# SaumikDana/Bayesian-Markov-chain-Monte-Carlo

Hardware: AMD Instinct MI355X
Metric: ode_steps_x_chains_per_sec (higher is better)
Workload: dtype f64

## Files before the change

### bayesian-markov-chain-monte-carlo_amd/csrc/rsf_device.h

```cpp
#pragma once
#include <hip/hip_runtime.h>
#include <stdint.h>

#include <type_traits>

#include "rsf_math.h"

namespace rsf {

struct Consts {
  double mu_ref, V_ref, k1, mu0;
  double a_def, b_def;
  double h, hh, h6;
  double inv_dt;
  double t0, dt;
  double inv_vref;
  double cacc;
  const double *vl;
  const double *data;
  int64_t group_chains;
  int32_t nout;
  int32_t S;
  int32_t kc;
  int32_t nchunks;
};

__device__ __forceinline__ void select_group(Consts &K) {
  if (K.group_chains > 0) K.data += ((int64_t)blockIdx.x * blockDim.x / K.group_chains) * K.nout;
}

struct Lane {
  double inv_dc;
  double vdc;
  double kprime;
  double kia;
  double khh, kh, kh6;
  double vk;
  double beta;
  double kvk;
  double vrw;
  double hhdw, hdw;
  double cv;
  double h6v;
  double boa;
  double nhboa;
  double tc;
  double hhd, hd, h6d;
  double bh;
  double c_l1p, c_l1q;
  double c_em1;
};

template <int T>
__device__ __forceinline__ void set_tier(Lane &L);

template <bool DAMP>
__device__ __forceinline__ Lane make_lane(double dc, double a, double b, const Consts &K) {
  Lane L;
  const double inv_a = fm::rcp(a);
  L.inv_dc = fm::rcp(dc);
  L.kprime = (1e-2 * 10) * L.inv_dc;
  L.kia = L.kprime * inv_a;
  L.khh = L.kia * K.hh;
  L.kh = L.kia * K.h;
  L.kh6 = L.kia * K.h6;
  const double via = K.V_ref * inv_a;
  L.vdc = K.V_ref * L.inv_dc;
  L.vk = via * L.kprime;
  L.beta = (b * K.V_ref) * (1.0 / (1e-2 * 10));
  L.kvk = K.k1 * via;
  const double ikw = DAMP ? fm::rcp(L.kvk) : 1.0;
  const double vkw = DAMP ? L.vk * ikw : L.vk;
  L.cv = K.cacc * vkw;
  L.h6v = K.h6 * vkw;
  L.boa = b * inv_a;
  L.tc = -K.mu_ref * inv_a;
  L.hhd = K.hh * L.vdc;
  L.hd = K.h * L.vdc;
  L.h6d = K.h6 * L.vdc;
  L.vrw = DAMP ? K.V_ref * ikw : K.V_ref;
  L.hhdw = DAMP ? L.hhd * ikw : L.hhd;
  L.hdw = DAMP ? L.hd * ikw : L.hd;
  L.nhboa = -0.5 * L.boa;
  L.bh = L.beta * fm::rcp(L.hhd);
  set_tier<2>(L);
  return L;
}


struct State {
  double ms, x, V;
  double w, rx;
};

template <bool DAMP>
__device__ __forceinline__ void rhs_tail(double w, double rx, double x, double vl, const Lane &L,
                                         const Consts &K, double &d0, double &d1, double &d2) {
  d1 = __builtin_fma(-w, x, 1.0);
  d0 = __builtin_fma(-K.V_ref, w, vl);
  const double bt = (L.beta * d1) * rx;
  double g = d0 - bt;
  if (DAMP) {
    const double kw = L.kvk * w;
    d0 = __builtin_fma(-kw, g, d0);
    g = d0 - bt;
    d2 = kw * g;
  } else {
    d2 = w * g;
  }
}

__device__ __forceinline__ void eval_full(double ms, double x, const Lane &L, const Consts &K, double &w, double &rx) {
  w = fm::exp(__builtin_fma(-L.boa, fm::log(x), __builtin_fma(ms, L.kia, L.tc)));
  rx = fm::rcp(x);
}

enum Tier : int { TIGHT = 0, NARROW = 1, WIDE = 2, FULL = 3 };

__device__ __forceinline__ double local_value(double x) {
  asm volatile("" : "+v"(x));
  return x;
}

template <bool DAMP, int T>
__device__ __forceinline__ void tier_enter(State &s, const Lane &L) {
  s.rx *= L.hhd;
  if (DAMP) s.w *= L.kvk;
}
template <int T>
__device__ __forceinline__ void tier_x(State &s, const Lane &L) { s.x = L.hhd * fm::rcp(s.rx); }
template <bool DAMP, int T>
__device__ __forceinline__ void tier_leave(State &s, const Lane &L) {
  tier_x<T>(s, L);
  s.rx *= fm::rcp(local_value(L.hhd));
  if (DAMP) s.w *= fm::rcp(local_value(L.kvk));
}
template <bool DAMP, int T>
__device__ __forceinline__ void eval_full_t(State &s, const Lane &L, const Consts &K) {
  eval_full(s.ms, s.x, L, K, s.w, s.rx);
  tier_enter<DAMP, T>(s, L);
}
template <bool DAMP, int T>
__device__ __forceinline__ void resync_t(State &s, const Lane &L, const Consts &K) {
  tier_x<T>(s, L);
  eval_full_t<DAMP, T>(s, L, K);
}


struct Guard {
  float rho, dlt;
  float dlt_h;
};

__device__ __forceinline__ float hi_as_float(double x) { return __builtin_bit_cast(float, __double2hiint(x)); }
constexpr float hi_pow2(int e) { return __builtin_bit_cast(float, (1023 + e) << 20); }


template <int T>
__device__ __forceinline__ void set_tier(Lane &L) {
  L.c_l1p = L.boa * (1.0 / 3.0);
  L.c_l1q = L.boa * (-1.0 / 4.0);
  L.c_em1 = T == TIGHT ? 1.0 / 24.0 : (T == NARROW ? 1.0 / 720.0 : 1.0 / 40320.0);
  asm volatile("" : "+v"(L.c_l1p), "+v"(L.c_l1q), "+v"(L.c_em1));
}

template <int T>
__device__ __forceinline__ bool guard_ok(const Guard &g) {
  return (g.rho < (T == WIDE ? hi_pow2(-11) : (T == NARROW ? hi_pow2(-14) : hi_pow2(-20)))) &&
         (g.dlt < (T == TIGHT ? hi_pow2(-9) : (T == NARROW ? hi_pow2(-7) : hi_pow2(-5)))) && (T != TIGHT || g.dlt_h < hi_pow2(-10));
}

constexpr float hi_pow2_34(int e) { return __builtin_bit_cast(float, ((1023 + e - 1) << 20) | 0x80000); }
template <int T>
__device__ __forceinline__ bool calm_enough(const Guard &g) {
  static_assert(T == NARROW || T == WIDE, "TIGHT has no tighter tier");
  return T == WIDE ? (g.rho < hi_pow2_34(-14) && g.dlt < hi_pow2_34(-7))
                   : (g.rho < hi_pow2_34(-20) && g.dlt < hi_pow2_34(-10));
}

constexpr int kResync = 512;

template <bool DAMP>
__device__ __forceinline__ double rk4_cold(State &s, double vl0, double vlm, double vl1, const Lane &L,
                                           const Consts &K) {
  double k0 = 0.0, k1 = 0.0, s0 = 0.0, s1 = 0.0, s2 = 0.0;
#pragma nounroll
  for (int st = 0; st < 4; ++st) {
    const double c = st == 0 ? 0.0 : (st == 3 ? K.h : K.hh);
    const double wgt = (st == 0 || st == 3) ? 1.0 : 2.0;
    const double vl = st == 0 ? vl0 : (st == 3 ? vl1 : vlm);
    const double x1 = __builtin_fma(c * L.vdc, k1, s.x);
    double w, rx, d0, d1, d2;
    eval_full(__builtin_fma(c, k0, s.ms), x1, L, K, w, rx);
    rhs_tail<DAMP>(w, rx, x1, vl, L, K, d0, d1, d2);
    s0 = __builtin_fma(wgt, d0, s0);
    s1 = __builtin_fma(wgt, d1, s1);
    s2 = __builtin_fma(wgt, d2, s2);
    k0 = d0;
    k1 = d1;
  }
  s.ms = __builtin_fma(K.h6, s0, s.ms);
  s.x = __builtin_fma(L.h6d, s1, s.x);
  return s2;
}

template <int T, bool HALF>
__device__ __forceinline__ void tight_incr(double rho, double dk, const Lane &L, double w0, double &w, double &q, Guard &g) {
  g.rho = __builtin_fmaxf(g.rho, __builtin_fabsf(hi_as_float(rho)));
  double pb = L.nhboa;
  if (T == NARROW) pb = __builtin_fma(rho, L.c_l1p, pb);
  if (T == WIDE) pb = __builtin_fma(rho, __builtin_fma(rho, L.c_l1q, L.c_l1p), pb);
  const double dlt = __builtin_fma(-rho, __builtin_fma(rho, pb, L.boa), dk);
  if (T == TIGHT && HALF) g.dlt_h = __builtin_fmaxf(g.dlt_h, __builtin_fabsf(hi_as_float(dlt)));
  else g.dlt = __builtin_fmaxf(g.dlt, __builtin_fabsf(hi_as_float(dlt)));
  double e = L.c_em1;
  if (T == WIDE) {
    e = fm::hfma(e, dlt, 1.0 / 5040.0);
    e = fm::hfma(e, dlt, 1.0 / 720.0);
  }
  if (T != TIGHT) {
    e = fm::hfma(e, dlt, 1.0 / 120.0);
    e = fm::hfma(e, dlt, 1.0 / 24.0);
  }
  e = fm::hfma(e, dlt, 1.0 / 6.0);
  e = __builtin_fma(e, dlt, 0.5);
  e = __builtin_fma(e, dlt, 1.0);
  w = __builtin_fma(w0 * dlt, e, w0);
  const double r1 = __builtin_fma(rho, rho, -rho);
  q = r1;
  if (T != TIGHT) q = __builtin_fma(-rho, q, -rho);
  if (T == WIDE) q = __builtin_fma(-rho, q, -rho);
}

template <bool DAMP>
__device__ __forceinline__ void rhs_tight(double w, double xr, double Rh, double vl, double brx, double vr, double &d0, double &d1,
                                          double &g) {
  d1 = __builtin_fma(-w, xr, Rh);
  d0 = __builtin_fma(-vr, w, vl);
  g = __builtin_fma(-brx, d1, d0);
  if (DAMP) {
    d0 = __builtin_fma(-w, g, d0);
    g = __builtin_fma(-w, g, g);
  }
}

template <bool DAMP, int T>
__device__ __forceinline__ double rk4_tight(State &s, double vl0, double vlm, double vl1, const Lane &L, const Consts &K, Guard &g) {
  double a0, a1, a2, b0, b1, b2, c0, c1, c2, e0, e1, e2, w, q;
  const double Rh = s.rx;
  const double vr = L.vrw, xh = L.hhdw, xf = L.hdw;
  rhs_tight<DAMP>(s.w, xh, Rh, vl0, L.bh, vr, a0, a1, a2);
  double sv = s.w * a2;
  tight_incr<T, true>(a1, L.khh * a0, L, s.w, w, q, g);
  rhs_tight<DAMP>(w, __builtin_fma(xh, a1, xh), Rh, vlm, __builtin_fma(L.bh, q, L.bh), vr, b0, b1, b2);
  double sm = w * b2;
  tight_incr<T, true>(b1, L.khh * b0, L, s.w, w, q, g);
  rhs_tight<DAMP>(w, __builtin_fma(xh, b1, xh), Rh, vlm, __builtin_fma(L.bh, q, L.bh), vr, c0, c1, c2);
  sm = __builtin_fma(w, c2, sm);
  tight_incr<T, false>(c1 + c1, L.kh * c0, L, s.w, w, q, g);
  rhs_tight<DAMP>(w, __builtin_fma(xf, c1, xh), Rh, vl1, __builtin_fma(L.bh, q, L.bh), vr, e0, e1, e2);
  sv = __builtin_fma(w, e2, sv);
  const double t0 = a0 + 2.0 * b0 + 2.0 * c0 + e0;
  const double t1 = a1 + 2.0 * b1 + 2.0 * c1 + e1;
  const double rho = t1 * (1.0 / 3.0);
  tight_incr<T, false>(rho, L.kh6 * t0, L, s.w, w, q, g);
  s.ms = __builtin_fma(K.h6, t0, s.ms);
  s.w = w;
  s.rx = __builtin_fma(Rh, q, Rh);
  return __builtin_fma(2.0, sm, sv);
}

__device__ __forceinline__ State initial_state(double dc, const Lane &L, const Consts &K) {
  State s;
  s.ms = (K.mu0 * dc) * (1.0 / (1e-2 * 10));
  s.x = K.V_ref * ((dc * K.inv_vref) * L.inv_dc);
  s.V = K.V_ref;
  eval_full(s.ms, s.x, L, K, s.w, s.rx);
  return s;
}

constexpr int kLdsPad = 0;
__device__ __forceinline__ int lds_data_offset(const Consts &K) { return 2 * K.S * K.kc + 1 + kLdsPad; }
__device__ __forceinline__ int lds_d0_offset(const Consts &K) { return lds_data_offset(K) + K.kc; }

__device__ __forceinline__ void stage_chunk(double *lds, const Consts &K, int k0, int kn) {
  const int nv = 2 * K.S * kn + 1;
  const int base = 2 * K.S * (k0 - 1);
  __syncthreads();
  for (int i = threadIdx.x; i < nv; i += blockDim.x) lds[i] = K.vl[base + i];
  if (K.data) {
    double *ld = lds + lds_data_offset(K);
    for (int i = threadIdx.x; i < kn; i += blockDim.x) ld[i] = K.data[k0 + i];
    if (threadIdx.x == 0) lds[lds_d0_offset(K)] = K.data[0];
  }
  __syncthreads();
}

struct Emit {
  int ko;
  int phase;
  double vprev;
};

template <bool WANT_SSQ, bool WANT_ACC>
__device__ __forceinline__ void emit_at(double vnow, double vprev, int ko, double obs, const Consts &K, int k0,
                                        double &ssq, bool active, double *acc_out, int64_t stride) {
  const double ak = (vnow - vprev) * K.inv_dt;
  if (WANT_ACC && active) acc_out[(int64_t)(k0 + ko) * stride] = ak;
  if (WANT_SSQ) {
    const double r = ak - obs;
    ssq = __builtin_fma(r, r, ssq);
  }
}

template <bool WANT_SSQ, bool WANT_ACC>
__device__ __forceinline__ void emit_incr(double dvs, int ko, double obs, const Lane &L, int k0, double &ssq,
                                          bool active, double *acc_out, int64_t stride) {
  if (WANT_ACC && active) acc_out[(int64_t)(k0 + ko) * stride] = dvs * L.cv;
  if (WANT_SSQ) {
    const double r = __builtin_fma(dvs, L.cv, -obs);
    ssq = __builtin_fma(r, r, ssq);
  }
}

template <bool WANT_SSQ, bool WANT_ACC>
__device__ __forceinline__ void emit_sample(double vnow, Emit &em, double obs, const Consts &K, int k0, double &ssq,
                                            bool active, double *acc_out, int64_t stride) {
  emit_at<WANT_SSQ, WANT_ACC>(vnow, em.vprev, em.ko, obs, K, k0, ssq, active, acc_out, stride);
  em.vprev = vnow;
  ++em.ko;
}

template <bool DAMP, int T, int NU>
__device__ __forceinline__ bool trip_fast(const double *v, const Lane &L, const Consts &K, State &s, double (&dv)[NU], bool *calm = nullptr) {
  Guard g = {0, 0, 0};
#pragma unroll
  for (int j = 0; j < NU; ++j) dv[j] = rk4_tight<DAMP, T>(s, v[2 * j], v[2 * j + 1], v[2 * j + 2], L, K, g);
  if constexpr (T != TIGHT) {
    if (calm) *calm = calm_enough<T>(g);
  }
  return !guard_ok<T>(g);
}

template <bool DAMP, int T, int NU>
__device__ __forceinline__ void trip_cold(const double *v, const Lane &L, const Consts &K, State &s, double (&dv)[NU]) {
  tier_x<T>(s, L);
#pragma unroll 1
  for (int j = 0; j < NU; ++j) {
    const double r = rk4_cold<DAMP>(s, v[2 * j], v[2 * j + 1], v[2 * j + 2], L, K);
#pragma unroll
    for (int m = 0; m < NU; ++m) dv[m] = m == j ? r : dv[m];
  }
  eval_full_t<DAMP, T>(s, L, K);
}

template <bool DAMP, int NU>
__device__ __forceinline__ void trip_cold_plain(const double *v, const Lane &L, const Consts &K, State &s, double (&dv)[NU]) {
#pragma unroll 1
  for (int j = 0; j < NU; ++j) {
    const double r = rk4_cold<DAMP>(s, v[2 * j], v[2 * j + 1], v[2 * j + 2], L, K);
#pragma unroll
    for (int m = 0; m < NU; ++m) dv[m] = m == j ? r : dv[m];
  }
  eval_full(s.ms, s.x, L, K, s.w, s.rx);
}

constexpr int kFullRetry = 32;
constexpr int kCalmSteps = 16;
struct Wave {
  unsigned long long alive;
  unsigned long long need[3];
  unsigned long long stiff;
  int next_resync;
  int full_run;
  int calm;
  uint32_t steps[4], redone, lane_steps;
};

__device__ __forceinline__ unsigned long long ballot(bool p) { return __builtin_amdgcn_ballot_w64(p); }
__device__ __forceinline__ bool lane_in(unsigned long long mask) { return (mask >> (threadIdx.x & 63)) & 1; }
template <int CTRL>
__device__ __forceinline__ double dpp_move(double v) {
  const int lo = __builtin_amdgcn_update_dpp(0, __double2loint(v), CTRL, 0xF, 0xF, false);
  const int hi = __builtin_amdgcn_update_dpp(0, __double2hiint(v), CTRL, 0xF, 0xF, false);
  return __hiloint2double(hi, lo);
}

__device__ __forceinline__ void wave_begin(Wave &W, bool active, const Lane &L, const Consts &K) {
  const double dk = 1.2 * K.V_ref * K.h * L.kia;
  W.alive = ballot(active);
  W.need[0] = ballot(active && !(dk < 0x1.0p-9));
  W.need[1] = ballot(active && !(dk < 0x1.0p-7));
  W.need[2] = W.stiff = ballot(active && !(dk < 0x1.0p-3));
  W.next_resync = kResync;
  W.full_run = 0;
  W.calm = 0;
}

__device__ __forceinline__ int wave_tier(const Wave &W) {
  return (W.need[2] & W.alive) ? FULL : ((W.need[1] & W.alive) ? WIDE : ((W.need[0] & W.alive) ? NARROW : TIGHT));
}

template <bool WANT_SSQ, bool WANT_ACC, bool S1, int NU>
__device__ __forceinline__ void emit_trip(const double (&dv)[NU], const double (&obs)[NU], const double *ld, int r, State &s, Emit &em,
                                          const Lane &L, const Consts &K, int k0, double &ssq, bool active, double *acc_out, int64_t stride) {
  if (S1) {
#pragma unroll
    for (int j = 0; j < NU; ++j) emit_incr<WANT_SSQ, WANT_ACC>(dv[j], r + j, obs[j], L, k0, ssq, active, acc_out, stride);
  } else {
#pragma unroll
    for (int j = 0; j < NU; ++j) {
      s.V = __builtin_fma(L.h6v, dv[j], s.V);
      if (++em.phase == K.S) {
        em.phase = 0;
        const double o = WANT_SSQ ? ld[em.ko] : 0.0;
        emit_sample<WANT_SSQ, WANT_ACC>(s.V, em, o, K, k0, ssq, active, acc_out, stride);
      }
    }
  }
}

constexpr int kTightUnroll = 8;
constexpr int kNarrowUnroll = 8, kWiderUnroll = 4;
template <bool DAMP, bool WANT_SSQ, bool WANT_ACC, int T, bool S1, int NU>
__device__ __forceinline__ int integrate_multi(const double *lds, const double *ld, const Consts &K, Lane L, int k0, int kn, int r,
                                               int nsteps, State &s, Emit &em, double &ssq, double thr, bool active, double *acc_out,
                                               int64_t stride, Wave &W) {
  static_assert(NU >= 1 && (kResync % NU) == 0, "trip lengths divide the resync interval");
  set_tier<T>(L);
  for (; r + NU <= nsteps; r += NU) {
    const unsigned long long deadmask = WANT_SSQ ? ballot(ssq > thr) : 0ull;
    const double *v = lds + 2 * r;
    double obs[NU], dv[NU];
#pragma unroll
    for (int j = 0; j < NU; ++j) obs[j] = (WANT_SSQ && S1) ? ld[r + j] : 0.0;
    if (r >= W.next_resync) {
      resync_t<DAMP, T>(s, L, K);
      W.next_resync = (r & ~(kResync - 1)) + kResync;
    }
    const State save = s;
    bool calm = false;
    const bool bad = trip_fast<DAMP, T, NU>(v, L, K, s, dv, &calm);
    const unsigned long long badmask = ballot(bad) & W.alive;
    W.steps[T] += NU;
    W.lane_steps += NU * (uint32_t)__builtin_popcountll(W.alive);
    if constexpr (T != TIGHT) {
      W.calm = (ballot(!calm) & W.alive) == 0 ? W.calm + NU : 0;
    }
    if (__builtin_expect(badmask != 0, 0)) {
      if (lane_in(badmask)) {
        s = save;
        trip_cold<DAMP, T, NU>(v, L, K, s, dv);
      }
      W.need[T] |= badmask;
      W.redone += NU;
      W.full_run = 0;
      W.calm = 0;
    }
    emit_trip<WANT_SSQ, WANT_ACC, S1, NU>(dv, obs, ld, r, s, em, L, K, k0, ssq, active, acc_out, stride);
    W.alive &= ~deadmask;
    if constexpr (T != TIGHT) {
      if (W.calm >= kCalmSteps && badmask == 0) {
        W.need[T - 1] &= ~W.alive | W.stiff;
        W.calm = 0;
      }
    }
    if (badmask != 0 || W.alive == 0 || (T != TIGHT && (W.need[T - 1] & W.alive) == 0)) return r + NU;
  }
  return r;
}

template <bool DAMP, bool WANT_SSQ, bool WANT_ACC, bool S1>
__device__ __forceinline__ int integrate_full(const double *lds, const double *ld, const Consts &K, const Lane &L, int k0, int kn, int r,
                                              int nsteps, State &s, Emit &em, double &ssq, double thr, bool active, double *acc_out,
                                              int64_t stride, Wave &W) {
#pragma unroll 1
  for (; r < nsteps; ++r) {
    const unsigned long long deadmask = WANT_SSQ ? ballot(ssq > thr) : 0ull;
    const double *v = lds + 2 * r;
    const double obs[1] = {(WANT_SSQ && S1) ? ld[r] : 0.0};
    const double dv[1] = {rk4_cold<DAMP>(s, v[0], v[1], v[2], L, K)};
    W.steps[FULL] += 1;
    W.lane_steps += (uint32_t)__builtin_popcountll(W.alive);
    emit_trip<WANT_SSQ, WANT_ACC, S1, 1>(dv, obs, ld, r, s, em, L, K, k0, ssq, active, acc_out, stride);
    W.alive &= ~deadmask;
    if (++W.full_run >= kFullRetry) {
      W.need[2] &= W.stiff;
      W.full_run = 0;
    }
    if (W.alive == 0 || (W.need[2] & W.alive) == 0) return r + 1;
  }
  return r;
}

__device__ __forceinline__ int start_tier(const Lane &L, const Consts &K) {
  const double dk = 1.2 * K.V_ref * K.h * L.kia;
  return !__any(!(dk < 0x1.0p-9)) ? TIGHT : (!__any(!(dk < 0x1.0p-7)) ? NARROW : WIDE);
}

constexpr int kLockstepTrip = 8;
template <bool DAMP, typename OnSample, typename AfterTrip>
__device__ __forceinline__ void integrate_lockstep(double *lds, const Consts &K, const Lane &L, State &st, int kn, OnSample on_sample,
                                                   AfterTrip after_trip) {
  constexpr int NU = kLockstepTrip;
  static_assert(kResync % NU == 0, "the resync test looks at the first step of a trip");
  const int nsteps = K.S * kn;
  double dsum = 0.0;
  int phase = 0, ko = 0;
  int tier = start_tier(L, K);
  int r = 0;
  auto trip = [&](auto tier_tag, auto nu_tag) {
    constexpr int T = decltype(tier_tag)::value, NUT = decltype(nu_tag)::value;
    const double *v = lds + 2 * r;
    Lane Lt = L;
    set_tier<T>(Lt);
    const State save = st;
    double dv[NUT];
    tier_enter<DAMP, T>(st, Lt);
    const bool bad = trip_fast<DAMP, T, NUT>(v, Lt, K, st, dv);
    tier_leave<DAMP, T>(st, Lt);
    const bool any_bad = ballot(bad) != 0;
    if (__builtin_expect(any_bad, 0)) {
      if (bad) {
        st = save;
        trip_cold_plain<DAMP, NUT>(v, L, K, st, dv);
      }
    }
#pragma unroll
    for (int j = 0; j < NUT; ++j) {
      dsum += dv[j];
      if (++phase == K.S) {
        phase = 0;
        on_sample(dsum * L.cv, ko);
        dsum = 0.0;
        ++ko;
      }
    }
    return any_bad;
  };
  for (; r + NU <= nsteps; r += NU) {
    if ((r & (kResync - 1)) == 0) eval_full(st.ms, st.x, L, K, st.w, st.rx);
    bool any_bad;
    if (tier == TIGHT) any_bad = trip(std::integral_constant<int, TIGHT>{}, std::integral_constant<int, NU>{});
    else if (tier == NARROW) any_bad = trip(std::integral_constant<int, NARROW>{}, std::integral_constant<int, NU>{});
    else any_bad = trip(std::integral_constant<int, WIDE>{}, std::integral_constant<int, NU>{});
    if (any_bad && tier < WIDE) ++tier;
    after_trip();
  }
  for (; r < nsteps; ++r) {
    if ((r & (kResync - 1)) == 0) eval_full(st.ms, st.x, L, K, st.w, st.rx);
    trip(std::integral_constant<int, WIDE>{}, std::integral_constant<int, 1>{});
    after_trip();
  }
}

template <bool DAMP, bool WANT_SSQ, bool WANT_ACC, int T, bool S1, int NU>
__device__ __forceinline__ int integrate_tier(const double *lds, const double *ld, const Consts &K, const Lane &L, int k0, int kn, int r,
                                              int nsteps, State &s, Emit &em, double &ssq, double thr, bool active, double *acc_out,
                                              int64_t stride, Wave &W) {
  if (r + NU <= nsteps) return integrate_multi<DAMP, WANT_SSQ, WANT_ACC, T, S1, NU>(lds, ld, K, L, k0, kn, r, nsteps, s, em, ssq, thr, active, acc_out, stride, W);
  return integrate_multi<DAMP, WANT_SSQ, WANT_ACC, T, S1, 2>(lds, ld, K, L, k0, kn, r, nsteps, s, em, ssq, thr, active, acc_out, stride, W);
}

template <bool DAMP, bool WANT_SSQ, bool WANT_ACC, bool S1, int NUT>
__device__ __forceinline__ void integrate_tiers(const double *lds, const double *ld, const Consts &K, const Lane &L, int k0,
                                                int kn, State &s, double &ssq, double thr, bool active, double *acc_out, int64_t stride, Wave &W) {
  const int nsteps = S1 ? kn : K.S * kn;
  Emit em = {0, 0, s.V};
  int r = 0;
  W.next_resync = kResync;
  bool scaled = false;
  while (r < nsteps && W.alive != 0) {
    const int tier = wave_tier(W);
    if (tier == FULL) {
      if (scaled) { tier_leave<DAMP, WIDE>(s, L); scaled = false; }
      r = integrate_full<DAMP, WANT_SSQ, WANT_ACC, S1>(lds, ld, K, L, k0, kn, r, nsteps, s, em, ssq, thr, active, acc_out, stride, W);
      eval_full(s.ms, s.x, L, K, s.w, s.rx);
      continue;
    }
    if (!scaled) { tier_enter<DAMP, TIGHT>(s, L); scaled = true; }
    if (nsteps - r == 1) r = integrate_multi<DAMP, WANT_SSQ, WANT_ACC, WIDE, S1, 1>(lds, ld, K, L, k0, kn, r, nsteps, s, em, ssq, thr, active, acc_out, stride, W);
    else if (tier == TIGHT) r = integrate_tier<DAMP, WANT_SSQ, WANT_ACC, TIGHT, S1, NUT>(lds, ld, K, L, k0, kn, r, nsteps, s, em, ssq, thr, active, acc_out, stride, W);
    else if (tier == NARROW) r = integrate_tier<DAMP, WANT_SSQ, WANT_ACC, NARROW, S1, kNarrowUnroll>(lds, ld, K, L, k0, kn, r, nsteps, s, em, ssq, thr, active, acc_out, stride, W);
    else r = integrate_tier<DAMP, WANT_SSQ, WANT_ACC, WIDE, S1, kWiderUnroll>(lds, ld, K, L, k0, kn, r, nsteps, s, em, ssq, thr, active, acc_out, stride, W);
  }
  if (scaled) tier_leave<DAMP, WIDE>(s, L);
}

template <bool DAMP, bool WANT_SSQ, bool WANT_ACC, int NUT>
__device__ __forceinline__ void integrate_chunk(const double *lds, const Consts &K, const Lane &L, int k0, int kn, State &s,
                                                double &ssq, double thr, bool active, double *acc_out, int64_t stride, Wave &W) {
  const double *ld = lds + lds_data_offset(K);
  if (K.S == 1) integrate_tiers<DAMP, WANT_SSQ, WANT_ACC, true, NUT>(lds, ld, K, L, k0, kn, s, ssq, thr, active, acc_out, stride, W);
  else integrate_tiers<DAMP, WANT_SSQ, WANT_ACC, false, NUT>(lds, ld, K, L, k0, kn, s, ssq, thr, active, acc_out, stride, W);
}

template <bool DAMP, bool WANT_SSQ, bool WANT_ACC, int NUT = kTightUnroll>
__device__ __forceinline__ double solve(double *lds, const Consts &K, bool resident, bool active, double dc, double a,
                                        double b, double thr, double *acc_out, int64_t stride, Wave &W) {
  const Lane L = make_lane<DAMP>(dc, a, b, K);
  State s = initial_state(dc, L, K);
  wave_begin(W, active, L, K);
  double ssq = 0.0;
  if (WANT_ACC && active) acc_out[0] = 0.0;
  for (int k0 = 1; k0 < K.nout; k0 += K.kc) {
    const int kn = min(K.kc, K.nout - k0);
    if (!resident) stage_chunk(lds, K, k0, kn);
    if (WANT_SSQ && k0 == 1) {
      const double d0 = lds[lds_d0_offset(K)];
      ssq = d0 * d0;
    }
    if (W.alive != 0) integrate_chunk<DAMP, WANT_SSQ, WANT_ACC, NUT>(lds, K, L, k0, kn, s, ssq, thr, active, acc_out, stride, W);
  }
  return ssq;
}

enum : uint32_t { SLOT_Z01 = 0, SLOT_Z2 = 1, SLOT_U = 2, SLOT_GAMMA = 8 };

__device__ __forceinline__ void philox4x32_10(uint32_t c0, uint32_t c1, uint32_t c2, uint32_t c3, uint32_t k0,
                                              uint32_t k1, uint32_t out[4]) {
#pragma unroll
  for (int r = 0; r < 10; ++r) {
    const uint32_t hi0 = __umulhi(0xD2511F53u, c0), lo0 = 0xD2511F53u * c0;
    const uint32_t hi1 = __umulhi(0xCD9E8D57u, c2), lo1 = 0xCD9E8D57u * c2;
    const uint32_t n0 = hi1 ^ c1 ^ k0, n2 = hi0 ^ c3 ^ k1;
    c0 = n0; c1 = lo1; c2 = n2; c3 = lo0;
    k0 += 0x9E3779B9u;
    k1 += 0xBB67AE85u;
  }
  out[0] = c0; out[1] = c1; out[2] = c2; out[3] = c3;
}

__device__ __forceinline__ void draw_words(uint64_t seed, uint64_t chain, uint32_t iter, uint32_t slot,
                                           uint32_t w[4]) {
  philox4x32_10((uint32_t)chain, (uint32_t)(chain >> 32), iter, slot, (uint32_t)seed, (uint32_t)(seed >> 32), w);
}

__device__ __forceinline__ double u53(uint32_t hi, uint32_t lo) {
  const uint64_t k = (((uint64_t)hi << 32) | lo) >> 11;
  return (double)(k + 1) * 0x1.0p-53;
}

__device__ __forceinline__ void normal_pair(const uint32_t w[4], double &z0, double &z1) {
  const double u1 = u53(w[0], w[1]), u2 = u53(w[2], w[3]);
  const double r = sqrt(-2.0 * fm::log(u1));
  double s, c;
  fm::sincos2pi(u2, s, c);
  z0 = r * c;
  z1 = r * s;
}

__device__ __forceinline__ double rng_log(double x) { return fm::log(x); }

__device__ __forceinline__ double gamma_draw(uint64_t seed, uint64_t chain, uint32_t iter, double d, double c) {
  for (uint32_t j = 0; j < 64; ++j) {
    uint32_t w[4];
    double x, unused;
    draw_words(seed, chain, iter, SLOT_GAMMA + 2 * j, w);
    normal_pair(w, x, unused);
    double v = 1.0 + c * x;
    if (!(v > 0.0)) continue;
    v = v * v * v;
    draw_words(seed, chain, iter, SLOT_GAMMA + 2 * j + 1, w);
    const double u = u53(w[0], w[1]);
    if (rng_log(u) < 0.5 * x * x + d * (1.0 - v + rng_log(v))) return d * v;
  }
  return d;
}

template <int D>
__device__ __forceinline__ bool chol_lower(const double *V, double *L) {
  bool ok = true;
#pragma unroll
  for (int e = 0; e < D * D; ++e) L[e] = 0.0;
#pragma unroll
  for (int j = 0; j < D; ++j) {
    double s = V[j * D + j];
#pragma unroll
    for (int k = 0; k < j; ++k) s -= L[j * D + k] * L[j * D + k];
    if (!(s > 0.0)) { ok = false; continue; }
    const double ljj = sqrt(s);
    L[j * D + j] = ljj;
#pragma unroll
    for (int i = j + 1; i < D; ++i) {
      double t = V[i * D + j];
#pragma unroll
      for (int k = 0; k < j; ++k) t -= L[i * D + k] * L[j * D + k];
      L[i * D + j] = t / ljj;
    }
  }
  return ok;
}

template <int D>
__device__ __forceinline__ void sym_inverse(const double *A, double *Ai) {
  if (D == 1) {
    Ai[0] = 1.0 / A[0];
  } else {
    const double c00 = A[4] * A[8] - A[5] * A[7], c01 = A[5] * A[6] - A[3] * A[8], c02 = A[3] * A[7] - A[4] * A[6];
    const double id = 1.0 / (A[0] * c00 + A[1] * c01 + A[2] * c02);
    Ai[0] = c00 * id; Ai[1] = (A[2] * A[7] - A[1] * A[8]) * id; Ai[2] = (A[1] * A[5] - A[2] * A[4]) * id;
    Ai[3] = c01 * id; Ai[4] = (A[0] * A[8] - A[2] * A[6]) * id; Ai[5] = (A[2] * A[3] - A[0] * A[5]) * id;
    Ai[6] = c02 * id; Ai[7] = (A[1] * A[6] - A[0] * A[7]) * id; Ai[8] = (A[0] * A[4] - A[1] * A[3]) * id;
  }
}

template <int D>
__device__ __forceinline__ bool window_covariance(const double *ws, const double *wq, double nn, double scale, const double *eps, double *Vn,
                                                  double *Ln) {
#pragma unroll
  for (int p = 0; p < D; ++p)
#pragma unroll
    for (int r = 0; r < D; ++r) Vn[p * D + r] = scale * ((wq[p * D + r] - ws[p] * ws[r] / nn) / (nn - 1.0) + (p == r ? eps[p] : 0.0));
  return chol_lower<D>(Vn, Ln);
}

template <typename F>
__device__ __forceinline__ double np_cov_1d(F a, int n) {
  double sum;
  if (n < 8) {
    sum = 0.0;
    for (int i = 0; i < n; ++i) sum += a(i);
  } else {
    double r[8];
#pragma unroll
    for (int j = 0; j < 8; ++j) r[j] = a(j);
    int i = 8;
    for (; i < n - (n % 8); i += 8)
#pragma unroll
      for (int j = 0; j < 8; ++j) r[j] += a(i + j);
    sum = ((r[0] + r[1]) + (r[2] + r[3])) + ((r[4] + r[5]) + (r[6] + r[7]));
    for (; i < n; ++i) sum += a(i);
  }
  const double avg = sum / (double)n;
  double c = 0.0;
  for (int k = 0; k < n; ++k) {
    const double dlt = a(k) - avg;
    c = __builtin_fma(dlt, dlt, c);
  }
  return c * (1.0 / (double)(n - 1));
}

}
```

### bayesian-markov-chain-monte-carlo_amd/csrc/rsf_kernels_sampler.h

```cpp
#pragma once
#include <hip/hip_runtime.h>
#include <stdint.h>

#include <type_traits>

#include "rsf_kernel_common.h"
#include "rsf_device_dop853.h"
#include "rsf_device_f32.h"

namespace rsfk {

constexpr int kD3Trip = 2;

constexpr int kFlushEvery = 16;
constexpr int kProposalTries = 4;
struct WaveCounters {
  uint32_t accepted, evaluated, nonfinite, oob, early, wave_solves, wave_skips;
  rsf::Wave W;
  __device__ __forceinline__ void reset() {
    accepted = evaluated = nonfinite = oob = early = wave_solves = wave_skips = 0;
    W.steps[0] = W.steps[1] = W.steps[2] = W.steps[3] = W.redone = W.lane_steps = 0;
  }
  __device__ __forceinline__ void flush(unsigned long long *stats) {
    if ((threadIdx.x & 63) == 0) {
// ... 26 lines not shown
  static_assert(MODE == RK4_F64 || MODE == DOP853, "the float32 sampler is mcmc_f32x2_kernel (two chains per lane)");
  static_assert(!INJECT || REPLAY, "supplied sums of squares come with supplied variates");
  extern __shared__ __attribute__((aligned(16))) double lds[];
  rsf::select_group(K);
  const int64_t blk = (int64_t)blockIdx.x * blockDim.x;
  const unsigned t = threadIdx.x;
  const int64_t i = blk + t;
  const bool valid = i < A.C;
  auto at = [&](auto *base, int e) { return base + ((int64_t)e * A.C + blk); };
  const bool resident = K.nchunks == 1;

  double q[D];
  double ssq = 0.0, std2 = 1.0;
#pragma unroll
  for (int p = 0; p < D; ++p) q[p] = 1.0;
  double *lcs = lds + A.lc_off + t;
  double V1 = 0.0;
  double wr[D], ws[D], wq[D * D];
  int32_t wn = 0;
  auto store_factor = [&](const double *Lf) {
    int e = 0;
#pragma unroll
    for (int p = 0; p < D; ++p)
#pragma unroll
      for (int r = 0; r <= p; ++r) lcs[(e++) * blockDim.x] = Lf[p * D + r];
  };
  if (valid) {
#pragma unroll
    for (int p = 0; p < D; ++p) q[p] = at(A.q, p)[t];
    ssq = at(A.ssq, 0)[t];
    std2 = at(A.std2, 0)[t];
  }
  if constexpr (D == 1) {
    if (valid) V1 = at(A.V, 0)[t];
  } else {
    double V[D * D], Lf[D * D];
#pragma unroll
    for (int e = 0; e < D * D; ++e) V[e] = valid ? at(A.V, e)[t] : 0.0;
    rsf::chol_lower<D>(V, Lf);
    store_factor(Lf);
  }
  auto load_window = [&](unsigned t) {
#pragma unroll
    for (int p = 0; p < D; ++p) { wr[p] = at(A.wref, p)[t]; ws[p] = at(A.wsum, p)[t]; }
#pragma unroll
    for (int e = 0; e < D * D; ++e) wq[e] = at(A.wsq, e)[t];
    wn = at(A.wn, 0)[t];
  };
  auto store_window = [&](unsigned t) {
#pragma unroll
    for (int p = 0; p < D; ++p) { at(A.wref, p)[t] = wr[p]; at(A.wsum, p)[t] = ws[p]; }
#pragma unroll
    for (int e = 0; e < D * D; ++e) at(A.wsq, e)[t] = wq[e];
    at(A.wn, 0)[t] = wn;
  };
  WaveCounters cnt;
  cnt.reset();

  if (resident && !INJECT) {
    if constexpr (MODE == DOP853) rsf::dp::stage_chunk_dp(lds, K, 1, K.nout - 1);
    else rsf::stage_chunk(lds, K, 1, K.nout - 1);
  }

  constexpr bool kPark = MODE == RK4_F64;
  constexpr int kSlotQ = factor_slots(D), kSlotStd2 = kSlotQ + D, kSlotSsq = kSlotStd2 + 1, kSlotLu = kSlotSsq + 1;
  static_assert(kSlotLu + 1 == park_slots(D), "rsf_sampler.hip sizes the launch's LDS with park_slots");

#pragma unroll
  for (int p = 0; p < D; ++p) asm volatile("" : "+v"(q[p]));
  asm volatile("" : "+v"(ssq), "+v"(std2), "+v"(V1));
  const int32_t n_iters = (int32_t)A.n_iters;
  const int max_tries = (REPLAY || !resident) ? 1 : kProposalTries;
  int32_t nl = valid ? 0 : n_iters;
  int32_t to_adapt = A.adapt_interval - (int32_t)(A.iter_base % A.adapt_interval);
  bool have = false;
  double qn[D], lu = 0.0, thr = INFINITY;
#pragma unroll
  for (int p = 0; p < D; ++p) qn[p] = 1.0;
  int tries = 0;
  for (int32_t round = 0;; ++round) {
    const bool todo = nl < n_iters;
    if (resident ? !__any(todo) : round == n_iters) break;
    const uint32_t it = (uint32_t)(A.iter_base + nl);
    unsigned tl = t;
    asm volatile("" : "+v"(tl));
    const uint64_t gid = (uint64_t)(A.chain_offset + blk + tl);
    const int64_t row = (int64_t)nl * A.C + blk + tl;
    if (todo && !have) {
      double z[4] = {0.0, 0.0, 0.0, 0.0};
      if (REPLAY) {
#pragma unroll
        for (int p = 0; p < D; ++p) z[p] = A.z[row * D + p];
      } else {
        uint32_t w[4];
        rsf::draw_words(A.seed, gid, it, rsf::SLOT_Z01, w);
        rsf::normal_pair(w, z[0], z[1]);
        if (D > 2) {
          rsf::draw_words(A.seed, gid, it, rsf::SLOT_Z2, w);
          rsf::normal_pair(w, z[2], z[3]);
        }
      }
      if constexpr (D == 1) {
        double Lc;
        rsf::chol_lower<1>(&V1, &Lc);
        propose<1>(q, [&](int) { return Lc; }, z, qn);
      } else {
        propose<D>(q, [&](int e) { return lcs[e * blockDim.x]; }, z, qn);
      }
      have = in_box<D>(qn, A);
      lu = 0.0;
      thr = INFINITY;
      if (have) {
        double u;
        if (REPLAY) {
          u = A.u[row];
        } else {
          uint32_t w[4];
          rsf::draw_words(A.seed, gid, it, rsf::SLOT_U, w);
          u = rsf::u53(w[0], w[1]);
        }
        lu = REPLAY ? log(u) : rsf::rng_log(u);
        if constexpr (MODE == RK4_F64 && !INJECT) {
          const double t0 = __builtin_fma(-2.0 * std2, lu, ssq);
          thr = __builtin_fma(1e-9, __builtin_fabs(t0), t0);
        }
      }
    }
    const bool oob = todo && !have;
    const bool solve_now = tries + 1 >= max_tries || !__any(oob);
    tries = solve_now ? 0 : tries + 1;
    double ssqn = 0.0;
    if (solve_now) {
      const unsigned long long inbmask = rsf::ballot(have);
      cnt.evaluated += (uint32_t)__builtin_popcountll(inbmask);
      if constexpr (!INJECT) {
        if (inbmask != 0) ++cnt.wave_solves;
        else ++cnt.wave_skips;
      }
      if constexpr (kPark) {
#pragma unroll
        for (int p = 0; p < D; ++p) lcs[(kSlotQ + p) * blockDim.x] = q[p];
        lcs[kSlotStd2 * blockDim.x] = std2;
        lcs[kSlotSsq * blockDim.x] = ssq;
        lcs[kSlotLu * blockDim.x] = lu;
      }
      double an = K.a_def, bn = K.b_def;
      if constexpr (D == 3) { an = qn[1]; bn = qn[2]; }
      if constexpr (INJECT) {
        if (have) ssqn = A.ssq_new[row];
      } else if (!resident || inbmask != 0) {
        if constexpr (MODE == DOP853) {
          ssqn = rsf::dp::solve<DAMP, true, false>(lds, K, resident, have, qn[0], an, bn, nullptr, 0);
        } else {
          ssqn = rsf::solve<DAMP, true, false, (D == 1 ? 2 : kD3Trip) * rsf::kTightUnroll>(lds, K, resident, have, qn[0], an, bn, thr, nullptr, 0, cnt.W);
          cnt.early += (uint32_t)__builtin_popcountll(inbmask & ~cnt.W.alive);
        }
      }
      if constexpr (kPark) {
        unsigned relaunder = 0;
        asm volatile("" : "+v"(relaunder));
        const double *back = lcs + relaunder;
#pragma unroll
        for (int p = 0; p < D; ++p) q[p] = back[(kSlotQ + p) * blockDim.x];
        std2 = back[kSlotStd2 * blockDim.x];
        ssq = back[kSlotSsq * blockDim.x];
        lu = back[kSlotLu * blockDim.x];
      }
    }
    const bool solved = solve_now && have;
    bool accept = false;
    if (solved) {
      accept = metropolis<REPLAY>(ssq, ssqn, std2, lu);
      if (accept) {
        ssq = ssqn;
#pragma unroll
        for (int p = 0; p < D; ++p) q[p] = qn[p];
      }
    }
    cnt.accepted += (uint32_t)__builtin_popcountll(rsf::ballot(accept));
    cnt.nonfinite += (uint32_t)__builtin_popcountll(rsf::ballot(solved && !isfinite(ssqn)));
    cnt.oob += (uint32_t)__builtin_popcountll(rsf::ballot(oob));
    if (solved || oob) {
      std2 = gibbs_std2<REPLAY>(A, gid, it, row, 0, std2, ssq);
      if (A.tq) {
#pragma unroll
        for (int p = 0; p < D; ++p) A.tq[row * D + p] = q[p];
      }
      if (A.ts) A.ts[row] = std2;
      if (A.ta) A.ta[row] = accept ? 1 : 0;
      if (A.adapt_mode != RSF_ADAPT_NONE) {
        load_window(tl);
#pragma unroll
        for (int p = 0; p < D; ++p) {
          ws[p] += q[p] - wr[p];
#pragma unroll
          for (int r = 0; r < D; ++r) wq[p * D + r] += (q[p] - wr[p]) * (q[r] - wr[r]);
        }
        ++wn;
        if (A.adapt_mode == RSF_ADAPT_REFERENCE_DICT) at(A.wbuf, A.adapt_interval - to_adapt)[tl] = q[0];
        if (--to_adapt == 0) {
          to_adapt = A.adapt_interval;
          if (wn >= 2) {
            const double nn = (double)wn;
            double Vn[D * D], Ln[D * D];
            if (A.adapt_mode == RSF_ADAPT_REFERENCE_DICT) {
              Vn[0] = A.dict_scale * rsf::np_cov_1d([&](int k) { return at(A.wbuf, k)[tl]; }, A.adapt_interval);
              if (rsf::chol_lower<1>(Vn, Ln)) V1 = Ln[0];
            } else if (rsf::window_covariance<D>(ws, wq, nn, 2.38 * 2.38 / (double)D, A.am_eps, Vn, Ln)) {
              if constexpr (D == 1) {
                V1 = Vn[0];
              } else {
#pragma unroll
                for (int e = 0; e < D * D; ++e) at(A.V, e)[tl] = Vn[e];
                store_factor(Ln);
              }
            }
          }
        }
        store_window(tl);
      }
      ++nl;
      have = false;
    }
    if ((round & (kFlushEvery - 1)) == kFlushEvery - 1) cnt.flush(A.stats);
  }

  if (valid) {
#pragma unroll
    for (int p = 0; p < D; ++p) at(A.q, p)[t] = q[p];
    if constexpr (D == 1) at(A.V, 0)[t] = V1;
    at(A.ssq, 0)[t] = ssq;
    at(A.std2, 0)[t] = std2;
  }
  cnt.flush(A.stats);
}

template <int D>
struct Chain {
  double q[D], ssq, std2;
  double V1;
  double wr[D], ws[D], wq[D * D];
  int32_t wn;
  bool valid;
  uint64_t gid;
};

template <int D, bool DAMP, bool REPLAY>
__global__ void __launch_bounds__(kMaxBlock, kMinBlocks) __attribute__((amdgpu_num_vgpr(RSF_F32_TRIP_COMPILER_VGPRS / 2)))
mcmc_f32x2_kernel(Consts K, McmcArgs A) {
  extern __shared__ __attribute__((aligned(16))) double lds[];
  constexpr int NC = 2;
  const int64_t blk = (int64_t)blockIdx.x * blockDim.x * NC;
  if (K.group_chains > 0) K.data += (blk / K.group_chains) * K.nout;
  const unsigned t = threadIdx.x;
  auto at = [&](auto *base, int e, int s) { return base + ((int64_t)e * A.C + blk + (int64_t)s * blockDim.x); };
  const bool resident = K.nchunks == 1;

  constexpr bool kWinRegs = D == 1;
  double *lcs = lds + A.lc_off + t;
  Chain<D> ch[NC];
  auto store_factor = [&](int s, const double *Lf) {
    int e = 0;
#pragma unroll
    for (int p = 0; p < D; ++p)
#pragma unroll
      for (int r = 0; r <= p; ++r) lcs[((e++) * NC + s) * blockDim.x] = Lf[p * D + r];
  };
  auto load_window = [&](int s, unsigned t) {
    Chain<D> &c = ch[s];
#pragma unroll
    for (int p = 0; p < D; ++p) { c.wr[p] = at(A.wref, p, s)[t]; c.ws[p] = at(A.wsum, p, s)[t]; }
#pragma unroll
    for (int e = 0; e < D * D; ++e) c.wq[e] = at(A.wsq, e, s)[t];
    c.wn = at(A.wn, 0, s)[t];
  };
  auto store_window = [&](int s, unsigned t) {
    const Chain<D> &c = ch[s];
#pragma unroll
    for (int p = 0; p < D; ++p) { at(A.wref, p, s)[t] = c.wr[p]; at(A.wsum, p, s)[t] = c.ws[p]; }
#pragma unroll
    for (int e = 0; e < D * D; ++e) at(A.wsq, e, s)[t] = c.wq[e];
    at(A.wn, 0, s)[t] = c.wn;
  };
#pragma unroll
  for (int s = 0; s < NC; ++s) {
    Chain<D> &c = ch[s];
    const int64_t i = blk + (int64_t)s * blockDim.x + t;
    c.valid = i < A.C;
    c.gid = (uint64_t)(A.chain_offset + i);
    c.ssq = 0.0; c.std2 = 1.0; c.V1 = 0.0; c.wn = 0;
#pragma unroll
    for (int p = 0; p < D; ++p) c.q[p] = 1.0;
    if (c.valid) {
#pragma unroll
      for (int p = 0; p < D; ++p) c.q[p] = at(A.q, p, s)[t];
      c.ssq = at(A.ssq, 0, s)[t];
      c.std2 = at(A.std2, 0, s)[t];
    }
    if constexpr (D == 1) {
      if (c.valid) c.V1 = at(A.V, 0, s)[t];
    } else {
      double V[D * D], Lf[D * D];
#pragma unroll
      for (int e = 0; e < D * D; ++e) V[e] = c.valid ? at(A.V, e, s)[t] : 0.0;
      rsf::chol_lower<D>(V, Lf);
      store_factor(s, Lf);
    }
// ... 181 lines not shown
```

Before: 395.0 billion.

## Fold sum-of-squares residual into tight RK4 step and trim tight series

Adds an in-step variant of the tight RK4 path that computes the residual against the observation and accumulates the sum of squares inside the step, instead of returning per-step slip values and emitting them afterwards. The half-step exponential series is shortened by one term, and the final stage uses a specialised doubled-increment helper with precomputed lane constants. A new guard on the doubled stage is added, and the cold fallback recomputes the sum of squares directly. The aim is fewer live registers and fewer instructions per step, at the cost of a slightly different accuracy guard and extra template instantiations.

```diff
diff --git a/bayesian-markov-chain-monte-carlo_amd/csrc/rsf_device.h b/bayesian-markov-chain-monte-carlo_amd/csrc/rsf_device.h
--- a/bayesian-markov-chain-monte-carlo_amd/csrc/rsf_device.h
+++ b/bayesian-markov-chain-monte-carlo_amd/csrc/rsf_device.h
@@ -49,6 +49,9 @@
   double bh;
   double c_l1p, c_l1q;
   double c_em1;
+  double cv2;
+  double boa2;
+  double bh2, bh4;
 };
 
 template <int T>
@@ -83,6 +86,10 @@
   L.hdw = DAMP ? L.hd * ikw : L.hd;
   L.nhboa = -0.5 * L.boa;
   L.bh = L.beta * fm::rcp(L.hhd);
+  L.cv2 = 2.0 * L.cv;
+  L.boa2 = 2.0 * L.boa;
+  L.bh2 = -2.0 * L.bh;
+  L.bh4 = 4.0 * L.bh;
   set_tier<2>(L);
   return L;
 }
@@ -150,6 +157,7 @@
 struct Guard {
   float rho, dlt;
   float dlt_h;
+  float rho_f;
 };
 
 __device__ __forceinline__ float hi_as_float(double x) { return __builtin_bit_cast(float, __double2hiint(x)); }
@@ -204,8 +212,9 @@
   return s2;
 }
 
-template <int T, bool HALF>
+template <int T, bool HALF, bool SHORT = false>
 __device__ __forceinline__ void tight_incr(double rho, double dk, const Lane &L, double w0, double &w, double &q, Guard &g) {
+  static_assert(!SHORT || (T == TIGHT && HALF), "the short series is for TIGHT's half-step stages");
   g.rho = __builtin_fmaxf(g.rho, __builtin_fabsf(hi_as_float(rho)));
   double pb = L.nhboa;
   if (T == NARROW) pb = __builtin_fma(rho, L.c_l1p, pb);
@@ -213,7 +222,7 @@
   const double dlt = __builtin_fma(-rho, __builtin_fma(rho, pb, L.boa), dk);
   if (T == TIGHT && HALF) g.dlt_h = __builtin_fmaxf(g.dlt_h, __builtin_fabsf(hi_as_float(dlt)));
   else g.dlt = __builtin_fmaxf(g.dlt, __builtin_fabsf(hi_as_float(dlt)));
-  double e = L.c_em1;
+  double e = SHORT ? 1.0 / 6.0 : L.c_em1;
   if (T == WIDE) {
     e = fm::hfma(e, dlt, 1.0 / 5040.0);
     e = fm::hfma(e, dlt, 1.0 / 720.0);
@@ -222,7 +231,7 @@
     e = fm::hfma(e, dlt, 1.0 / 120.0);
     e = fm::hfma(e, dlt, 1.0 / 24.0);
   }
-  e = fm::hfma(e, dlt, 1.0 / 6.0);
+  if (!SHORT) e = fm::hfma(e, dlt, 1.0 / 6.0);
   e = __builtin_fma(e, dlt, 0.5);
   e = __builtin_fma(e, dlt, 1.0);
   w = __builtin_fma(w0 * dlt, e, w0);
@@ -230,6 +239,17 @@
   q = r1;
   if (T != TIGHT) q = __builtin_fma(-rho, q, -rho);
   if (T == WIDE) q = __builtin_fma(-rho, q, -rho);
+}
+
+__device__ __forceinline__ void tight_incr_doubled(double c1, double dk, const Lane &L, double w0, double &w, double &brx, Guard &g) {
+  g.rho_f = __builtin_fmaxf(g.rho_f, __builtin_fabsf(hi_as_float(c1)));
+  const double dlt = __builtin_fma(-c1, __builtin_fma(-c1, L.boa2, L.boa2), dk);
+  g.dlt = __builtin_fmaxf(g.dlt, __builtin_fabsf(hi_as_float(dlt)));
+  double e = fm::hfma(L.c_em1, dlt, 1.0 / 6.0);
+  e = __builtin_fma(e, dlt, 0.5);
+  e = __builtin_fma(e, dlt, 1.0);
+  w = __builtin_fma(w0 * dlt, e, w0);
+  brx = __builtin_fma(c1, __builtin_fma(c1, L.bh4, L.bh2), L.bh);
 }
 
 template <bool DAMP>
@@ -244,21 +264,29 @@
   }
 }
 
-template <bool DAMP, int T>
-__device__ __forceinline__ double rk4_tight(State &s, double vl0, double vlm, double vl1, const Lane &L, const Consts &K, Guard &g) {
+template <bool DAMP, int T, bool INSTEP = false>
+__device__ __forceinline__ double rk4_tight(State &s, double vl0, double vlm, double vl1, const Lane &L, const Consts &K, Guard &g,
+                                            double obs = 0.0, double *ssq = nullptr, bool first = false) {
+  static_assert(!INSTEP || T == TIGHT, "the in-step sum of squares is the TIGHT step's");
   double a0, a1, a2, b0, b1, b2, c0, c1, c2, e0, e1, e2, w, q;
   const double Rh = s.rx;
   const double vr = L.vrw, xh = L.hhdw, xf = L.hdw;
   rhs_tight<DAMP>(s.w, xh, Rh, vl0, L.bh, vr, a0, a1, a2);
   double sv = s.w * a2;
-  tight_incr<T, true>(a1, L.khh * a0, L, s.w, w, q, g);
+  tight_incr<T, true, INSTEP>(a1, L.khh * a0, L, s.w, w, q, g);
   rhs_tight<DAMP>(w, __builtin_fma(xh, a1, xh), Rh, vlm, __builtin_fma(L.bh, q, L.bh), vr, b0, b1, b2);
   double sm = w * b2;
-  tight_incr<T, true>(b1, L.khh * b0, L, s.w, w, q, g);
+  tight_incr<T, true, INSTEP>(b1, L.khh * b0, L, s.w, w, q, g);
   rhs_tight<DAMP>(w, __builtin_fma(xh, b1, xh), Rh, vlm, __builtin_fma(L.bh, q, L.bh), vr, c0, c1, c2);
   sm = __builtin_fma(w, c2, sm);
-  tight_incr<T, false>(c1 + c1, L.kh * c0, L, s.w, w, q, g);
-  rhs_tight<DAMP>(w, __builtin_fma(xf, c1, xh), Rh, vl1, __builtin_fma(L.bh, q, L.bh), vr, e0, e1, e2);
+  if constexpr (INSTEP) {
+    double brx;
+    tight_incr_doubled(c1, L.kh * c0, L, s.w, w, brx, g);
+    rhs_tight<DAMP>(w, __builtin_fma(xf, c1, xh), Rh, vl1, brx, vr, e0, e1, e2);
+  } else {
+    tight_incr<T, false>(c1 + c1, L.kh * c0, L, s.w, w, q, g);
+    rhs_tight<DAMP>(w, __builtin_fma(xf, c1, xh), Rh, vl1, __builtin_fma(L.bh, q, L.bh), vr, e0, e1, e2);
+  }
   sv = __builtin_fma(w, e2, sv);
   const double t0 = a0 + 2.0 * b0 + 2.0 * c0 + e0;
   const double t1 = a1 + 2.0 * b1 + 2.0 * c1 + e1;
@@ -267,6 +295,11 @@
   s.ms = __builtin_fma(K.h6, t0, s.ms);
   s.w = w;
   s.rx = __builtin_fma(Rh, q, Rh);
+  if constexpr (INSTEP) {
+    const double r = __builtin_fma(sv, L.cv, __builtin_fma(sm, L.cv2, -obs));
+    *ssq = first ? r * r : __builtin_fma(r, r, *ssq);
+    return 0.0;
+  }
   return __builtin_fma(2.0, sm, sv);
 }
 
@@ -333,7 +366,7 @@
 
 template <bool DAMP, int T, int NU>
 __device__ __forceinline__ bool trip_fast(const double *v, const Lane &L, const Consts &K, State &s, double (&dv)[NU], bool *calm = nullptr) {
-  Guard g = {0, 0, 0};
+  Guard g = {0, 0, 0, 0};
 #pragma unroll
   for (int j = 0; j < NU; ++j) dv[j] = rk4_tight<DAMP, T>(s, v[2 * j], v[2 * j + 1], v[2 * j + 2], L, K, g);
   if constexpr (T != TIGHT) {
@@ -350,6 +383,17 @@
     const double r = rk4_cold<DAMP>(s, v[2 * j], v[2 * j + 1], v[2 * j + 2], L, K);
 #pragma unroll
     for (int m = 0; m < NU; ++m) dv[m] = m == j ? r : dv[m];
+  }
+  eval_full_t<DAMP, T>(s, L, K);
+}
+
+template <bool DAMP, int T, int NU>
+__device__ __forceinline__ void trip_cold_ssq(const double *v, const double *ob, const Lane &L, const Consts &K, State &s, double &ssq) {
+  tier_x<T>(s, L);
+#pragma unroll 1
+  for (int j = 0; j < NU; ++j) {
+    const double dvs = rk4_cold<DAMP>(s, v[2 * j], v[2 * j + 1], v[2 * j + 2], L, K);
+    emit_incr<true, false>(dvs, j, ob[j], L, 0, ssq, false, nullptr, 0);
   }
   eval_full_t<DAMP, T>(s, L, K);
 }
@@ -401,6 +445,15 @@
   return (W.need[2] & W.alive) ? FULL : ((W.need[1] & W.alive) ? WIDE : ((W.need[0] & W.alive) ? NARROW : TIGHT));
 }
 
+template <bool DAMP, int NU>
+__device__ __forceinline__ unsigned long long trip_fast_ssq(const double *v, const double (&obs)[NU], const Lane &L, const Consts &K, State &s,
+                                                            double &tsum) {
+  Guard g = {0, 0, 0, 0};
+#pragma unroll
+  for (int j = 0; j < NU; ++j) rk4_tight<DAMP, TIGHT, true>(s, v[2 * j], v[2 * j + 1], v[2 * j + 2], L, K, g, obs[j], &tsum, j == 0);
+  return ballot(!(g.rho < hi_pow2(-20))) | ballot(!(g.rho_f < hi_pow2(-21))) | ballot(!(g.dlt < hi_pow2(-9))) | ballot(!(g.dlt_h < hi_pow2(-10)));
+}
+
 template <bool WANT_SSQ, bool WANT_ACC, bool S1, int NU>
 __device__ __forceinline__ void emit_trip(const double (&dv)[NU], const double (&obs)[NU], const double *ld, int r, State &s, Emit &em,
                                           const Lane &L, const Consts &K, int k0, double &ssq, bool active, double *acc_out, int64_t stride) {
@@ -422,16 +475,17 @@
 
 constexpr int kTightUnroll = 8;
 constexpr int kNarrowUnroll = 8, kWiderUnroll = 4;
-template <bool DAMP, bool WANT_SSQ, bool WANT_ACC, int T, bool S1, int NU>
+template <bool DAMP, bool WANT_SSQ, bool WANT_ACC, int T, bool S1, int NU, bool INSTEP = false>
 __device__ __forceinline__ int integrate_multi(const double *lds, const double *ld, const Consts &K, Lane L, int k0, int kn, int r,
                                                int nsteps, State &s, Emit &em, double &ssq, double thr, bool active, double *acc_out,
                                                int64_t stride, Wave &W) {
   static_assert(NU >= 1 && (kResync % NU) == 0, "trip lengths divide the resync interval");
+  static_assert(!INSTEP || (T == TIGHT && WANT_SSQ && !WANT_ACC && S1), "the in-step sum of squares: TIGHT, SSq alone, one step per sample");
   set_tier<T>(L);
   for (; r + NU <= nsteps; r += NU) {
     const unsigned long long deadmask = WANT_SSQ ? ballot(ssq > thr) : 0ull;
     const double *v = lds + 2 * r;
-    double obs[NU], dv[NU];
+    double obs[NU], dv[INSTEP ? 1 : NU];
 #pragma unroll
     for (int j = 0; j < NU; ++j) obs[j] = (WANT_SSQ && S1) ? ld[r + j] : 0.0;
     if (r >= W.next_resync) {
@@ -440,8 +494,11 @@
     }
     const State save = s;
     bool calm = false;
-    const bool bad = trip_fast<DAMP, T, NU>(v, L, K, s, dv, &calm);
-    const unsigned long long badmask = ballot(bad) & W.alive;
+    double tsum = 0.0;
+    unsigned long long tripped;
+    if constexpr (INSTEP) tripped = trip_fast_ssq<DAMP, NU>(v, obs, L, K, s, tsum);
+    else tripped = ballot(trip_fast<DAMP, T, NU>(v, L, K, s, dv, &calm));
+    const unsigned long long badmask = tripped & W.alive;
     W.steps[T] += NU;
     W.lane_steps += NU * (uint32_t)__builtin_popcountll(W.alive);
     if constexpr (T != TIGHT) {
@@ -450,14 +507,20 @@
     if (__builtin_expect(badmask != 0, 0)) {
       if (lane_in(badmask)) {
         s = save;
-        trip_cold<DAMP, T, NU>(v, L, K, s, dv);
+        if constexpr (INSTEP) {
+          tsum = 0.0;
+          trip_cold_ssq<DAMP, T, NU>(v, ld + r, L, K, s, ssq);
+        } else {
+          trip_cold<DAMP, T, NU>(v, L, K, s, dv);
+        }
       }
       W.need[T] |= badmask;
       W.redone += NU;
       W.full_run = 0;
       W.calm = 0;
     }
-    emit_trip<WANT_SSQ, WANT_ACC, S1, NU>(dv, obs, ld, r, s, em, L, K, k0, ssq, active, acc_out, stride);
+    if constexpr (INSTEP) ssq += tsum;
+    else emit_trip<WANT_SSQ, WANT_ACC, S1, NU>(dv, obs, ld, r, s, em, L, K, k0, ssq, active, acc_out, stride);
     W.alive &= ~deadmask;
     if constexpr (T != TIGHT) {
       if (W.calm >= kCalmSteps && badmask == 0) {
@@ -554,17 +617,18 @@
   }
 }
 
-template <bool DAMP, bool WANT_SSQ, bool WANT_ACC, int T, bool S1, int NU>
+template <bool DAMP, bool WANT_SSQ, bool WANT_ACC, int T, bool S1, int NU, bool INSTEP = false>
 __device__ __forceinline__ int integrate_tier(const double *lds, const double *ld, const Consts &K, const Lane &L, int k0, int kn, int r,
                                               int nsteps, State &s, Emit &em, double &ssq, double thr, bool active, double *acc_out,
                                               int64_t stride, Wave &W) {
-  if (r + NU <= nsteps) return integrate_multi<DAMP, WANT_SSQ, WANT_ACC, T, S1, NU>(lds, ld, K, L, k0, kn, r, nsteps, s, em, ssq, thr, active, acc_out, stride, W);
-  return integrate_multi<DAMP, WANT_SSQ, WANT_ACC, T, S1, 2>(lds, ld, K, L, k0, kn, r, nsteps, s, em, ssq, thr, active, acc_out, stride, W);
-}
-
-template <bool DAMP, bool WANT_SSQ, bool WANT_ACC, bool S1, int NUT>
+  if (r + NU <= nsteps) return integrate_multi<DAMP, WANT_SSQ, WANT_ACC, T, S1, NU, INSTEP>(lds, ld, K, L, k0, kn, r, nsteps, s, em, ssq, thr, active, acc_out, stride, W);
+  return integrate_multi<DAMP, WANT_SSQ, WANT_ACC, T, S1, 2, INSTEP>(lds, ld, K, L, k0, kn, r, nsteps, s, em, ssq, thr, active, acc_out, stride, W);
+}
+
+template <bool DAMP, bool WANT_SSQ, bool WANT_ACC, bool S1, int NUT, bool SSQ_IN_STEP>
 __device__ __forceinline__ void integrate_tiers(const double *lds, const double *ld, const Consts &K, const Lane &L, int k0,
                                                 int kn, State &s, double &ssq, double thr, bool active, double *acc_out, int64_t stride, Wave &W) {
+  constexpr bool INSTEP = SSQ_IN_STEP && WANT_SSQ && !WANT_ACC && S1;
   const int nsteps = S1 ? kn : K.S * kn;
   Emit em = {0, 0, s.V};
   int r = 0;
@@ -580,22 +644,22 @@
     }
     if (!scaled) { tier_enter<DAMP, TIGHT>(s, L); scaled = true; }
     if (nsteps - r == 1) r = integrate_multi<DAMP, WANT_SSQ, WANT_ACC, WIDE, S1, 1>(lds, ld, K, L, k0, kn, r, nsteps, s, em, ssq, thr, active, acc_out, stride, W);
-    else if (tier == TIGHT) r = integrate_tier<DAMP, WANT_SSQ, WANT_ACC, TIGHT, S1, NUT>(lds, ld, K, L, k0, kn, r, nsteps, s, em, ssq, thr, active, acc_out, stride, W);
+    else if (tier == TIGHT) r = integrate_tier<DAMP, WANT_SSQ, WANT_ACC, TIGHT, S1, NUT, INSTEP>(lds, ld, K, L, k0, kn, r, nsteps, s, em, ssq, thr, active, acc_out, stride, W);
     else if (tier == NARROW) r = integrate_tier<DAMP, WANT_SSQ, WANT_ACC, NARROW, S1, kNarrowUnroll>(lds, ld, K, L, k0, kn, r, nsteps, s, em, ssq, thr, active, acc_out, stride, W);
     else r = integrate_tier<DAMP, WANT_SSQ, WANT_ACC, WIDE, S1, kWiderUnroll>(lds, ld, K, L, k0, kn, r, nsteps, s, em, ssq, thr, active, acc_out, stride, W);
   }
   if (scaled) tier_leave<DAMP, WIDE>(s, L);
 }
 
-template <bool DAMP, bool WANT_SSQ, bool WANT_ACC, int NUT>
+template <bool DAMP, bool WANT_SSQ, bool WANT_ACC, int NUT, bool SSQ_IN_STEP>
 __device__ __forceinline__ void integrate_chunk(const double *lds, const Consts &K, const Lane &L, int k0, int kn, State &s,
                                                 double &ssq, double thr, bool active, double *acc_out, int64_t stride, Wave &W) {
   const double *ld = lds + lds_data_offset(K);
-  if (K.S == 1) integrate_tiers<DAMP, WANT_SSQ, WANT_ACC, true, NUT>(lds, ld, K, L, k0, kn, s, ssq, thr, active, acc_out, stride, W);
-  else integrate_tiers<DAMP, WANT_SSQ, WANT_ACC, false, NUT>(lds, ld, K, L, k0, kn, s, ssq, thr, active, acc_out, stride, W);
-}
-
-template <bool DAMP, bool WANT_SSQ, bool WANT_ACC, int NUT = kTightUnroll>
+  if (K.S == 1) integrate_tiers<DAMP, WANT_SSQ, WANT_ACC, true, NUT, SSQ_IN_STEP>(lds, ld, K, L, k0, kn, s, ssq, thr, active, acc_out, stride, W);
+  else integrate_tiers<DAMP, WANT_SSQ, WANT_ACC, false, NUT, SSQ_IN_STEP>(lds, ld, K, L, k0, kn, s, ssq, thr, active, acc_out, stride, W);
+}
+
+template <bool DAMP, bool WANT_SSQ, bool WANT_ACC, int NUT = kTightUnroll, bool SSQ_IN_STEP = false>
 __device__ __forceinline__ double solve(double *lds, const Consts &K, bool resident, bool active, double dc, double a,
                                         double b, double thr, double *acc_out, int64_t stride, Wave &W) {
   const Lane L = make_lane<DAMP>(dc, a, b, K);
@@ -610,7 +674,7 @@
       const double d0 = lds[lds_d0_offset(K)];
       ssq = d0 * d0;
     }
-    if (W.alive != 0) integrate_chunk<DAMP, WANT_SSQ, WANT_ACC, NUT>(lds, K, L, k0, kn, s, ssq, thr, active, acc_out, stride, W);
+    if (W.alive != 0) integrate_chunk<DAMP, WANT_SSQ, WANT_ACC, NUT, SSQ_IN_STEP>(lds, K, L, k0, kn, s, ssq, thr, active, acc_out, stride, W);
   }
   return ssq;
 }
diff --git a/bayesian-markov-chain-monte-carlo_amd/csrc/rsf_kernels_sampler.h b/bayesian-markov-chain-monte-carlo_amd/csrc/rsf_kernels_sampler.h
--- a/bayesian-markov-chain-monte-carlo_amd/csrc/rsf_kernels_sampler.h
+++ b/bayesian-markov-chain-monte-carlo_amd/csrc/rsf_kernels_sampler.h
@@ -202,7 +202,7 @@
         if constexpr (MODE == DOP853) {
           ssqn = rsf::dp::solve<DAMP, true, false>(lds, K, resident, have, qn[0], an, bn, nullptr, 0);
         } else {
-          ssqn = rsf::solve<DAMP, true, false, (D == 1 ? 2 : kD3Trip) * rsf::kTightUnroll>(lds, K, resident, have, qn[0], an, bn, thr, nullptr, 0, cnt.W);
+          ssqn = rsf::solve<DAMP, true, false, (D == 1 ? 2 : kD3Trip) * rsf::kTightUnroll, true>(lds, K, resident, have, qn[0], an, bn, thr, nullptr, 0, cnt.W);
           cnt.early += (uint32_t)__builtin_popcountll(inbmask & ~cnt.W.alive);
         }
       }
```

Result: faster. 408.5 billion, median of 6 (+3.4%).
